# Alexandre-nk-Perdereau/video-fingerprint

Hardware: NVIDIA B200
Metric: fingerprint videos/s (64 frames@64^2) (higher is better)
Workload: dtype bf16

## Files before the change

### video_fingerprint_b200/csrc/vfp_b200.cu

```cuda
#include "../../include/vfp_b200.h"

#include <math.h>
#include <string.h>

#include <map>
#include <mutex>
#include <string>
#include <vector>

#include "conv1_kernel.cuh"
#include "attention_tc_kernel.cuh"
#include "conv3_ts_kernel.cuh"
#include "ffn_kernel.cuh"
#include "gemm_launch.cuh"
#include "join_kernels.cuh"
#include "metrics_kernels.cuh"
#include "model3d_kernels.cuh"
#include "preprocess_kernels.cuh"
#include "stem_ts_kernel.cuh"
#include "token_kernels.cuh"
#include "topk_kernels.cuh"

using namespace vfp;

namespace {

thread_local std::string g_last_error;

int fail(const std::string& msg) {
  g_last_error = msg;
  return 1;
}
int fail_cuda(const char* what, cudaError_t e) {
  g_last_error = std::string(what) + ": " + cudaGetErrorString(e);
  return 2;
}
#define VFP_CUDA(call)                                  \
  do {                                                  \
    cudaError_t e__ = (call);                           \
    if (e__ != cudaSuccess) return fail_cuda(#call, e__); \
  } while (0)

inline size_t align_up(size_t x, size_t a) { return (x + a - 1) / a * a; }

constexpr float kBnEps = 1e-5f;

enum Stage : int {
  kStConv1 = 0, kStConv2, kStConv3, kStConv4, kStTokEmbed, kStTemporalConv, kStLayerNorm, kStQkv, kStAttention,
  kStOutProj, kStMlp1, kStMlp2, kStPoolGemm, kStPool, kStFinal, kStMisc, kStStemFused, kStFfn, kNumStages
};
const char* const kStageNames[kNumStages] = {"conv1_stem", "conv2_igemm", "conv3_igemm", "conv4_igemm_pool", "token_embed_gemm",
                                             "temporal_conv", "layernorm", "qkv_gemm", "attention", "out_proj_gemm",
                                             "mlp1_gemm_gelu", "mlp2_gemm", "pool_logits_gemm", "temporal_pool",
                                             "final_projection", "misc", "stem_fused", "ffn_fused"};
struct Profiler {
  bool enabled = false;
  std::vector<cudaEvent_t> pool;
  std::vector<std::pair<int, cudaEvent_t>> marks;
  size_t next = 0;
  double ms[kNumStages] = {0};
  unsigned long long launches = 0;
  void mark(int stage, cudaStream_t st) {
    if (!enabled) return;
    if (next == pool.size()) {
      cudaEvent_t e;
      cudaEventCreate(&e);
      pool.push_back(e);
    }
    cudaEvent_t e = pool[next++];
    cudaEventRecord(e, st);
    marks.emplace_back(stage, e);
  }
  void drain() {
    if (marks.empty()) return;
    cudaEventSynchronize(marks.back().second);
    for (size_t i = 1; i < marks.size(); ++i) {
      if (marks[i].first < 0) continue;
      float t = 0.f;
      cudaEventElapsedTime(&t, marks[i - 1].second, marks[i].second);
      ms[marks[i].first] += t;
    }
    marks.clear();
    next = 0;
  }
};
Profiler g_prof;
const int kTemporalKernels[4] = {3, 5, 7, 11};

struct Conv2KBlock { int c_half, dw, dh; };
const Conv2KBlock kConv2KBlocks[6] = {{1, 0, -1}, {0, 0, 0}, {1, 0, 0}, {1, -1, -1}, {0, -1, 0}, {1, -1, 0}};
inline int conv2_tap_index(int d, int sub) { return d == -1 ? (sub == 1 ? 0 : -1) : (sub == 0 ? 1 : 2); }

struct AttnBlockWeights {
  float *ln1_w, *ln1_b, *ln2_w, *ln2_b;
  __nv_bfloat16 *wqkv, *wo, *w1, *w2;
  float *bqkv, *bo, *b1, *b2;
  CUtensorMap tm_qkv, tm_o, tm_w1, tm_w2;
  CUtensorMap tm_qkv_h, tm_o_h;
  CUtensorMap tm_w1_ffn, tm_w2_ffn;
};

}

struct vfp_weights {
  int embedding_dim = 0;
  int n_attn = 0;
  std::vector<void*> allocs;
  uint32_t* c1_wpack = nullptr;
  float* c1_bias = nullptr;
  __nv_bfloat16 *c2_w = nullptr, *c3_w = nullptr, *c4_w = nullptr;
  float *c2_b = nullptr, *c3_b = nullptr, *c4_b = nullptr;
  CUtensorMap tm_c2, tm_c3, tm_c4;
  CUtensorMap tm_c3h, tm_c4h;
  __nv_bfloat16* c2f_w = nullptr;
  CUtensorMap tm_c2f;
  __nv_bfloat16* c1ts_w = nullptr;
  CUtensorMap tm_c1ts;
  __nv_bfloat16* wtok = nullptr;
  float* btok = nullptr;
  float* pe = nullptr;
  int pe_len = 0;
  CUtensorMap tm_tok;
  float* tc_w[2] = {nullptr, nullptr};
  float* tc_b[2] = {nullptr, nullptr};
  std::vector<AttnBlockWeights> attn;
  __nv_bfloat16* wpool = nullptr;
  float* bpool = nullptr;
  CUtensorMap tm_pool;
  float *w0t = nullptr, *b0 = nullptr, *w3t = nullptr, *b3 = nullptr;
  bool head_on_tensor_cores = false;
  __nv_bfloat16 *w0_bf = nullptr, *w3_bf = nullptr;
  CUtensorMap tm_head0, tm_head3;
};

namespace {

struct TensorTable {
// ... 11 lines not shown
    }
    return static_cast<const float*>(it->second->data);
  }
  bool has(const std::string& name) const { return by_name.count(name) != 0; }
  int64_t numel(const std::string& name) const {
    auto it = by_name.find(name);
    return it == by_name.end() ? -1 : it->second->numel;
  }
};

template <class T>
int upload(vfp_weights* w, const std::vector<T>& host, T** dev) {
  void* p = nullptr;
  VFP_CUDA(cudaMalloc(&p, host.size() * sizeof(T)));
  w->allocs.push_back(p);
  VFP_CUDA(cudaMemcpy(p, host.data(), host.size() * sizeof(T), cudaMemcpyHostToDevice));
  *dev = static_cast<T*>(p);
  return 0;
}

std::vector<__nv_bfloat16> to_bf16(const std::vector<float>& v) {
  std::vector<__nv_bfloat16> o(v.size());
  for (size_t i = 0; i < v.size(); ++i) o[i] = __float2bfloat16(v[i]);
  return o;
}

struct BnFold {
  std::vector<float> scale, shift;
};
bool load_bn(const TensorTable& t, const std::string& prefix, int c, BnFold* out, std::string* err) {
  const float* g = t.get(prefix + ".weight", c, err);
  const float* b = g ? t.get(prefix + ".bias", c, err) : nullptr;
  const float* m = b ? t.get(prefix + ".running_mean", c, err) : nullptr;
  const float* v = m ? t.get(prefix + ".running_var", c, err) : nullptr;
  if (!v) return false;
  out->scale.resize(c);
  out->shift.resize(c);
  for (int i = 0; i < c; ++i) {
    const double s = (double)g[i] / sqrt((double)v[i] + (double)kBnEps);
    out->scale[i] = (float)s;
    out->shift[i] = (float)((double)b[i] - (double)m[i] * s);
  }
  return true;
}

int prep_conv3x3(vfp_weights* w, const TensorTable& t, int conv_idx, int cin, int cout, __nv_bfloat16** dw, float** db,
                 std::string* err) {
  const std::string p = "spatial_encoder.encoder.";
  const float* cw = t.get(p + std::to_string(conv_idx) + ".weight", (int64_t)cout * cin * 9, err);
  const float* cb = cw ? t.get(p + std::to_string(conv_idx) + ".bias", cout, err) : nullptr;
  BnFold bn;
  if (!cb || !load_bn(t, p + std::to_string(conv_idx + 1), cout, &bn, err)) return 1;
  std::vector<float> wf((size_t)cout * 9 * cin), bf(cout);
  for (int co = 0; co < cout; ++co) {
    for (int c = 0; c < cin; ++c)
      for (int kh = 0; kh < 3; ++kh)
        for (int kw = 0; kw < 3; ++kw)
          wf[(size_t)co * 9 * cin + (kh * 3 + kw) * cin + c] = cw[(((size_t)co * cin + c) * 3 + kh) * 3 + kw] * bn.scale[co];
    bf[co] = cb[co] * bn.scale[co] + bn.shift[co];
  }
  if (upload(w, to_bf16(wf), dw) || upload(w, bf, db)) return 1;
  return 0;
}

int prep_dense_bf16(vfp_weights* w, const float* src, size_t n, __nv_bfloat16** dev) {
  std::vector<float> v(src, src + n);
  return upload(w, to_bf16(v), dev);
}
int prep_f32(vfp_weights* w, const float* src, size_t n, float** dev) {
  std::vector<float> v(src, src + n);
  return upload(w, v, dev);
}

constexpr int64_t kConvPassFrames = 262144;
constexpr int64_t kStemPassFrames = 16384;
int64_t g_conv_pass_frames = 65536;
int64_t g_stem_pass_frames = kStemPassFrames;
int g_fused_stem = 2;
int g_join_prefetch = 16;
int g_attention_tc = 1;
int g_conv3_ts = 1;
int g_pair_gemm = 1;
int g_ffn_mode = 1;
int g_conv_mcast = 0;
int g_join_kernel = 2;
int g_join_symmetric = 1;
int g_join_panel_tiles = 512;

struct TokenWs {
  size_t cu, att_items, tok_pos, tok_len, feat, xa, xb, xn, qkv, att, delta, delta2, h, logits, xbf, pooled, pooled_bf, head_h, total;
};
struct ConvWs {
  size_t c1, c2, c3, total;
};
TokenWs token_ws_layout(int64_t F, int64_t C) {
  TokenWs L{};
  size_t off = 0;
  auto take = [&](size_t bytes) {
    const size_t o = off;
    off = align_up(off + bytes, 1024);
    return o;
  };
  L.cu = take((size_t)(C + 1) * 4);
  L.att_items = take((size_t)(F / 64 + C + 1) * 16);
  L.tok_pos = take((size_t)F * 4);
  L.tok_len = take((size_t)F * 4);
  L.feat = take((size_t)F * 256 * 2);
  L.xa = take((size_t)F * kDim * 4);
  L.xb = take((size_t)F * kDim * 4);
  L.xn = take((size_t)F * kDim * 2);
  L.qkv = take((size_t)F * 3 * kDim * 2);
  L.att = take((size_t)F * kDim * 2);
  L.delta = take((size_t)F * kDim * 2);
  L.delta2 = take((size_t)F * kDim * 2);
  L.h = take((size_t)F * 4 * kDim * 2);
  L.logits = take((size_t)F * kDim * 4);
  L.xbf = take((size_t)F * kDim * 2);
  L.pooled = take((size_t)C * 3 * kDim * 4);
  L.pooled_bf = take((size_t)C * 3 * kDim * 2);
  L.head_h = take((size_t)C * kDim * 2);
  L.total = off;
  return L;
}
ConvWs conv_ws_layout(int64_t F) {
  ConvWs L{};
  size_t off = 0;
  auto take = [&](size_t bytes) {
    const size_t o = off;
    off = align_up(off + bytes, 1024);
    return o;
  };
  L.c1 = take((size_t)std::min<int64_t>(F, kStemPassFrames) * 32 * 32 * 32 * 2);
  L.c2 = take((size_t)F * 16 * 16 * 64 * 2);
  L.c3 = take((size_t)F * 8 * 8 * 128 * 2);
  L.total = off;
  return L;
}
size_t forward_ws_total(int64_t F, int64_t C) {
  return token_ws_layout(F, C).total + conv_ws_layout(std::min<int64_t>(F, g_conv_pass_frames)).total;
}

constexpr int kMaxPipes = 4;
int g_forward_pipes = 1;

int pipe_streams(int n, cudaStream_t* out) {
  static std::mutex mu;
  static cudaStream_t pool[kMaxDevices][kMaxPipes] = {};
  std::lock_guard<std::mutex> g(mu);
  const int dev = current_device();
  for (int i = 0; i < n; ++i) {
    if (!pool[dev][i]) VFP_CUDA(cudaStreamCreateWithFlags(&pool[dev][i], cudaStreamNonBlocking));
    out[i] = pool[dev][i];
  }
  return 0;
}

}

extern "C" {

int vfp_abi_version(void) { return VFP_ABI_VERSION; }
const char* vfp_last_error(void) { return g_last_error.c_str(); }

int vfp_device_sm_count(void) {
  int n = 0, dev = 0;
  if (cudaGetDeviceCount(&n) != cudaSuccess || n <= 0) return 0;
  if (cudaGetDevice(&dev) != cudaSuccess) return 0;
  int sms = 0;
  if (cudaDeviceGetAttribute(&sms, cudaDevAttrMultiProcessorCount, dev) != cudaSuccess) return 0;
  return sms;
}

int vfp_set_tuning(int key, long long value) {
  if (key == 0 && value >= 64 && value <= kStemPassFrames) { g_stem_pass_frames = value; return 0; }
  if (key == 1 && (value == 0 || value == 2)) { g_fused_stem = (int)value; return 0; }
  if (key == 5 && value >= 0 && value <= 4096) { g_join_prefetch = (int)value; return 0; }
  if (key == 6 && value >= 0 && value <= 4096) { g_topk_prefetch = (int)value; return 0; }
  if (key == 3 && value >= 64 && value <= kConvPassFrames) { g_conv_pass_frames = value; return 0; }
  if (key == 16 && value >= 0 && value <= 1) { g_conv3_ts = (int)value; return 0; }
  if (key == 17 && value >= 0 && value <= 1) { g_attention_tc = (int)value; return 0; }
  if (key == 15 && value >= 0 && value <= 3) { g_pair_gemm = (int)value; return 0; }
  if (key == 14 && value >= 0 && value <= 1) { g_ffn_mode = (int)value; return 0; }
  if (key == 13 && value >= 0 && value <= 3) { g_conv_mcast = (int)value; return 0; }
  if (key == 10 && value >= 0 && value <= 2) { g_join_kernel = (int)value; return 0; }
  if (key == 11 && value >= 0 && value <= 1) { g_join_symmetric = (int)value; return 0; }
  if (key == 12 && value >= 16 && value <= 65536) { g_join_panel_tiles = (int)value; return 0; }
  if (key == 7 && value >= 0 && value <= 1) { pdl_enabled().store((int)value); return 0; }
  if (key == 8 && value >= 0 && value <= 4096) { persistent_cta_limit().store((int)value); return 0; }
  if (key == 9 && value >= 1 && value <= kMaxPipes) { g_forward_pipes = (int)value; return 0; }
  if (key == 2) {
    const int mode = value != 0;
    const unsigned int zero = 0;
    if (cudaMemcpyToSymbol(g_vfp_hang_mode, &mode, sizeof(mode)) != cudaSuccess) return 2;
    if (cudaMemcpyToSymbol(g_vfp_hang_count, &zero, sizeof(zero)) != cudaSuccess) return 2;
    return 0;
  }
  return 1;
}

int vfp_profile_enable(int on) {
  g_prof.drain();
  g_prof.enabled = on != 0;
  return 0;
}
int vfp_profile_num_stages(void) { return kNumStages; }
const char* vfp_profile_stage_name(int i) { return (i >= 0 && i < kNumStages) ? kStageNames[i] : ""; }
int vfp_profile_read(double* stage_ms, int n_stages, uint64_t* launches, int reset) {
  g_prof.drain();
  for (int i = 0; i < n_stages && i < kNumStages; ++i) stage_ms[i] = g_prof.ms[i];
  if (launches) *launches = g_prof.launches;
  if (reset) {
    for (int i = 0; i < kNumStages; ++i) g_prof.ms[i] = 0;
    g_prof.launches = 0;
  }
  return 0;
}

unsigned int vfp_device_error_word(void) {
  unsigned int v = 0, zero = 0;
  cudaDeviceSynchronize();
  cudaMemcpyFromSymbol(&v, g_vfp_device_error, sizeof(v));
  if (v) cudaMemcpyToSymbol(g_vfp_device_error, &zero, sizeof(zero));
  return v;
}

#ifdef VFP_FFN_TRACE
int vfp_debug_ffn_trace(long long* out, int max_pairs) {
  (void)max_pairs;
  cudaDeviceSynchronize();
  cudaMemcpyFromSymbol(out, g_ffn_trace, sizeof(long long) * 8192 / 2);
  static long long zeros[4096];
  cudaMemcpyToSymbol(g_ffn_trace, zeros, sizeof(zeros));
  return 2048;
}
#endif

int vfp_debug_hang_log(unsigned int* out, int max_entries) {
  unsigned int n = 0;
  cudaDeviceSynchronize();
  if (cudaMemcpyFromSymbol(&n, g_vfp_hang_count, sizeof(n)) != cudaSuccess) return -1;
  if (n > 64) n = 64;
  if ((int)n > max_entries) n = (unsigned int)max_entries;
  if (n && cudaMemcpyFromSymbol(out, g_vfp_hang_log, (size_t)n * 16) != cudaSuccess) return -1;
  return (int)n;
}

void vfp_weights_destroy(vfp_weights* w) {
  if (!w) return;
  for (void* p : w->allocs) cudaFree(p);
  delete w;
}

int vfp_weights_embedding_dim(const vfp_weights* w) { return w ? w->embedding_dim : 0; }

int vfp_weights_create(const vfp_tensor_desc* tensors, int n_tensors, vfp_weights** out) {
  if (!tensors || !out) return fail("vfp_weights_create: null argument");
  if (vfp_device_sm_count() <= 0) return fail("vfp_weights_create: no CUDA device (there is no CPU fallback)");
  if (!tensor_map_encoder()) return fail("vfp_weights_create: cuTensorMapEncodeTiled not available from the driver");
  TensorTable t;
  for (int i = 0; i < n_tensors; ++i) t.by_name[tensors[i].name] = &tensors[i];
  std::string err;
  vfp_weights* w = new vfp_weights();
  auto bail = [&](const std::string& m) {
    vfp_weights_destroy(w);
    return fail("vfp_weights_create: " + (m.empty() ? g_last_error : m));
// ... 247 lines not shown
      for (int kb = 0; kb < 6; ++kb) {
        s.tap_c_blk[kb] = (signed char)kConv2KBlocks[kb].c_half;
        s.tap_w[kb] = (signed char)kConv2KBlocks[kb].dw;
        s.tap_h[kb] = (signed char)kConv2KBlocks[kb].dh;
      }
      EpiBiasActTma<true>::Params ep{};
      if (make_tmap_out(&ep.tmap_out, c2a + (size_t)s0 * 256 * 64, (uint64_t)n * 256, 64, true)) return fail("tensor map encode failed (conv2 out)");
      ep.bias = w->c2_b; ep.N = 64; ep.act = 1;
      VFP_CUDA((launch_gemm<64, 64, 3, EpiBiasActTma<true>, 3>(ta, w->tm_c2, s, ep, st)));
      g_prof.mark(kStConv2, st);
    }
  }
  g_prof.launches += 2;
  {
    if (g_conv3_ts) {
      Conv3Params cp{};
      if (make_tmap_nhwc_bf16(&cp.tmap_in, c2a, F, 16, 16, 64, 64, 8, 8, kC3Frames, 2) || make_tmap_out(&cp.tmap_out, c3a, (uint64_t)F * 64, 128, true))
        return fail("tensor map encode failed (conv3)");
      cp.w = w->c3_w; cp.bias = w->c3_b; cp.n_tiles = (int)((F + kC3Frames - 1) / kC3Frames);
      VFP_CUDA(ensure_dynamic_smem(reinterpret_cast<const void*>(conv3_ts_kernel<7>), Conv3Smem<7>::kTotal));
      VFP_CUDA(launch_kernel(conv3_ts_kernel<7>, dim3(std::min(cp.n_tiles, persistent_grid())), dim3(kC3Threads), Conv3Smem<7>::kTotal, st, cp));
      g_prof.mark(kStConv3, st);
    } else {
    if (make_tmap_nhwc_bf16(&ta, c2a, F, 16, 16, 64, 64, 8, 8, 2, 2)) return fail("tensor map encode failed (conv3)");
    GemmShape s{};
    s.m_tiles = (int)((F + 1) / 2); s.n_tiles = 1; s.k_blocks = 9; s.group_m = 16; s.a_conv = 1;
    s.tiles_per_frame = 1; s.frames_per_tile = 2; s.tile_out_rows = 8;
    conv_taps_strided(&s, 1);
    EpiConvTransposedTma::Params ep{};
    if (make_tmap_out(&ep.tmap_out, c3a, (uint64_t)F * 64, 128, true)) return fail("tensor map encode failed (conv3 out)");
    ep.bias = w->c3_b; ep.c_out = 128; ep.pixels_per_tile = 256;
    if (g_conv_mcast & 1) VFP_CUDA((launch_gemm<128, 64, 4, EpiConvTransposedTma, 2, true, 2>(ta, w->tm_c3h, s, ep, st)));
    else VFP_CUDA((launch_gemm<128, 64, 4, EpiConvTransposedTma, 2, true>(ta, w->tm_c3, s, ep, st)));
    g_prof.mark(kStConv3, st);
    }
  }
  {
    if (make_tmap_nhwc_bf16(&ta, c3a, F, 8, 8, 128, 64, 4, 4, 8, 2)) return fail("tensor map encode failed (conv4)");
    GemmShape s{};
    s.m_tiles = (int)((F + 7) / 8); s.n_tiles = 1; s.k_blocks = 18; s.group_m = 16; s.a_conv = 1;
    s.tiles_per_frame = 1; s.frames_per_tile = 8; s.tile_out_rows = 4;
    conv_taps_strided(&s, 2);
    EpiConvPool16::Params ep{};
    ep.bias = w->c4_b; ep.out_bf16 = feat_out; ep.frames = (int)F; ep.N = 256;
    if (g_pair_gemm & 1) VFP_CUDA((launch_gemm_pair<64, 6, EpiConvPool16>(ta, w->tm_c4h, s, ep, st)));
    else if (g_conv_mcast & 2) VFP_CUDA((launch_gemm<256, 64, 4, EpiConvPool16, 1, false, 2>(ta, w->tm_c4h, s, ep, st)));
    else VFP_CUDA((launch_gemm<256, 64, 4, EpiConvPool16>(ta, w->tm_c4, s, ep, st)));
    g_prof.mark(kStConv4, st);
  }
  return 0;
}

int forward_pass(const vfp_weights* w, const uint8_t* frames_base, int frame_dtype, size_t frame_bytes,
                 const int32_t* cu_host, int c0, int c1, float* emb_out, float* features_out, uint8_t* ws,
                 cudaStream_t st) {
  const int C = c1 - c0;
  const int64_t f0 = cu_host[c0];
  const int64_t F = cu_host[c1] - f0;
  const TokenWs L = token_ws_layout(F, C);
  uint8_t* conv_ws = ws + L.total;
  int* d_cu = reinterpret_cast<int*>(ws + L.cu);
  int* tok_pos = reinterpret_cast<int*>(ws + L.tok_pos);
  int* tok_len = reinterpret_cast<int*>(ws + L.tok_len);
  __nv_bfloat16* feat = reinterpret_cast<__nv_bfloat16*>(ws + L.feat);
  float* xa = reinterpret_cast<float*>(ws + L.xa);
  float* xb = reinterpret_cast<float*>(ws + L.xb);
  __nv_bfloat16* xn = reinterpret_cast<__nv_bfloat16*>(ws + L.xn);
  __nv_bfloat16* qkv = reinterpret_cast<__nv_bfloat16*>(ws + L.qkv);
  __nv_bfloat16* att = reinterpret_cast<__nv_bfloat16*>(ws + L.att);
  __nv_bfloat16* delta = reinterpret_cast<__nv_bfloat16*>(ws + L.delta);
  __nv_bfloat16* delta_f = reinterpret_cast<__nv_bfloat16*>(ws + L.delta2);
  __nv_bfloat16* hbuf = reinterpret_cast<__nv_bfloat16*>(ws + L.h);
  float* logits = reinterpret_cast<float*>(ws + L.logits);
  __nv_bfloat16* xbf = reinterpret_cast<__nv_bfloat16*>(ws + L.xbf);
  float* pooled = reinterpret_cast<float*>(ws + L.pooled);
  __nv_bfloat16* pooled_bf = reinterpret_cast<__nv_bfloat16*>(ws + L.pooled_bf);
  __nv_bfloat16* head_h = reinterpret_cast<__nv_bfloat16*>(ws + L.head_h);

  std::vector<int32_t> cu_rel(C + 1);
  int max_T = 0;
  for (int i = 0; i <= C; ++i) cu_rel[i] = (int32_t)(cu_host[c0 + i] - f0);
  for (int i = 0; i < C; ++i) max_T = std::max(max_T, cu_rel[i + 1] - cu_rel[i]);
  g_prof.mark(-1, st);
  g_prof.launches += 8 + 7 * (unsigned long long)w->n_attn;
  VFP_CUDA(cudaMemcpyAsync(d_cu, cu_rel.data(), (size_t)(C + 1) * 4, cudaMemcpyHostToDevice, st));
  std::vector<int32_t> items_host;
  items_host.reserve((size_t)(F / kAttRows + C) * 4);
  for (int i = 0; i < C; ++i)
    for (int q = cu_rel[i]; q < cu_rel[i + 1]; q += kAttRows) {
      items_host.push_back(q); items_host.push_back(cu_rel[i]); items_host.push_back(cu_rel[i + 1]); items_host.push_back(0);
    }
  const size_t n_items = items_host.size() / 4;
  int4* att_items = reinterpret_cast<int4*>(ws + L.att_items);
  VFP_CUDA(cudaMemcpyAsync(att_items, items_host.data(), items_host.size() * 4, cudaMemcpyHostToDevice, st));
  VFP_CUDA(launch_kernel(token_map_kernel, dim3((unsigned)((F + 255) / 256)), dim3(256), 0, st, d_cu, C, (int)F, tok_pos, tok_len));
  g_prof.mark(kStMisc, st);

  for (int64_t s0 = 0; s0 < F; s0 += g_conv_pass_frames) {
    const int64_t n = std::min<int64_t>(g_conv_pass_frames, F - s0);
    if (int rc = encode_frames_pass(w, frames_base + (size_t)(f0 + s0) * frame_bytes, frame_dtype, n, feat + s0 * 256, conv_ws, st))
      return rc;
  }
  auto token_gemm = [&](const __nv_bfloat16* A, int64_t M, int K, const CUtensorMap& tb, int N, const EpiBiasAct::Params& ep) -> int {
    CUtensorMap tma;
    if (make_tmap_rows_bf16(&tma, A, (uint64_t)M, (uint64_t)K, (uint64_t)K, 128, 64)) return fail("tensor map encode failed (tokens)");
    GemmShape s = plain_shape(M, N, K, 256, 64, 32);
    if (K == 256) {
      VFP_CUDA((launch_gemm_bres<256, 64, 4, 4, EpiBiasAct>(tma, tb, s, ep, st)));
    } else {
      VFP_CUDA((launch_gemm<256, 64, 4, EpiBiasAct>(tma, tb, s, ep, st)));
    }
    return 0;
  };
  auto token_gemm_bf16 = [&](const __nv_bfloat16* A, int64_t M, int K, const CUtensorMap& tb, int N, const float* bias, int act,
                             __nv_bfloat16* out, const CUtensorMap* tb_half = nullptr) -> int {
    CUtensorMap tma;
    if (make_tmap_rows_bf16(&tma, A, (uint64_t)M, (uint64_t)K, (uint64_t)K, 128, 64)) return fail("tensor map encode failed (tokens)");
    EpiBiasActTma<true>::Params ep{};
    if (make_tmap_out(&ep.tmap_out, out, (uint64_t)M, (uint64_t)N, true)) return fail("tensor map encode failed (token out)");
    ep.bias = bias; ep.N = N; ep.act = act;
    GemmShape s = plain_shape(M, N, K, 256, 64, 32);
    if (tb_half && (g_pair_gemm & 2)) {
      VFP_CUDA((launch_gemm_pair<64, 6, EpiBiasActTma<true>>(tma, *tb_half, s, ep, st)));
    } else if (K == 256) {
      VFP_CUDA((launch_gemm_bres<256, 64, 4, 4, EpiBiasActTma<true>>(tma, tb, s, ep, st)));
    } else {
      VFP_CUDA((launch_gemm<256, 64, 4, EpiBiasActTma<true>>(tma, tb, s, ep, st)));
    }
    return 0;
  };
  {
    CUtensorMap tma;
    if (make_tmap_rows_bf16(&tma, feat, (uint64_t)F, 256, 256, 128, 64)) return fail("tensor map encode failed (tokens)");
    EpiBiasActTma<false>::Params ep{};
    if (make_tmap_out(&ep.tmap_out, xa, (uint64_t)F, kDim, false)) return fail("tensor map encode failed (token embedding out)");
    ep.bias = w->btok; ep.N = kDim; ep.act = 0; ep.pe = w->pe; ep.token_pos = tok_pos; ep.M = (int)F;
    GemmShape s = plain_shape(F, kDim, 256, 256, 64, 32);
    VFP_CUDA((launch_gemm_bres<256, 64, 2, 4, EpiBiasActTma<false>>(tma, w->tm_tok, s, ep, st)));
    g_prof.mark(kStTokEmbed, st);
  }
  {
    VFP_CUDA(ensure_dynamic_smem(reinterpret_cast<const void*>(temporal_conv_tma_kernel), kTc2SmemBytes));
    float* bufs[3] = {xa, xb, xa};
    for (int blk = 0; blk < 2; ++blk) {
      TemporalConvParams tp{};
      if (make_tmap_rows_f32(&tp.tmap_x, bufs[blk], (uint64_t)F, kDim, kTc2Rows)) return fail("tensor map encode failed (temporal conv)");
      tp.tok_pos = tok_pos; tp.tok_len = tok_len; tp.w = w->tc_w[blk]; tp.bias = w->tc_b[blk]; tp.y = bufs[blk + 1];
      tp.n_tokens = (int)F; tp.n_tiles = (int)((F + kTc2Tok - 1) / kTc2Tok);
      const int grid = std::min(tp.n_tiles, 2 * persistent_grid());
      VFP_CUDA(launch_kernel(temporal_conv_tma_kernel, dim3((unsigned)grid), dim3(kTc2Threads), kTc2SmemBytes, st, tp));
    }
    g_prof.mark(kStTemporalConv, st);
  }
  const unsigned ln_grid = (unsigned)((F * 32 + 255) / 256);
  VFP_CUDA(ensure_dynamic_smem(reinterpret_cast<const void*>(attention_fa_kernel), kAttSmemBytes));
  AttnTcParams atc{};
  if (g_attention_tc) {
    if (make_tmap_rows_bf16(&atc.tmap_qkv, qkv, (uint64_t)F, 3 * kDim, 3 * kDim, 64, 64)) return fail("tensor map encode failed (attention)");
    atc.items = att_items; atc.out = att; atc.n_units = (int)n_items * 4;
    VFP_CUDA(ensure_dynamic_smem(reinterpret_cast<const void*>(attention_tc_kernel), kAtcSmemBytes));
  }
  for (int b = 0; b < w->n_attn; ++b) {
    const AttnBlockWeights& a = w->attn[b];
    VFP_CUDA(launch_kernel(add_layernorm_bf16_kernel, dim3(ln_grid), dim3(256), 0, st, xa, b > 0 ? delta : nullptr, b > 0 ? delta_f : nullptr, a.ln1_w, a.ln1_b, xn, (int)F, 1));
    g_prof.mark(kStLayerNorm, st);
    if (token_gemm_bf16(xn, F, kDim, a.tm_qkv, 3 * kDim, a.bqkv, 0, qkv, &a.tm_qkv_h)) return 1;
    g_prof.mark(kStQkv, st);
    if (g_attention_tc) {
      const int grid = std::min(atc.n_units, 2 * persistent_grid());
      VFP_CUDA(launch_kernel(attention_tc_kernel, dim3((unsigned)grid), dim3(kAtcThreads), kAtcSmemBytes, st, atc));
    } else {
      VFP_CUDA(launch_kernel(attention_fa_kernel, dim3((unsigned)n_items), dim3(kAttThreads), kAttSmemBytes, st, qkv, att_items, att, (int)F));
    }
    g_prof.mark(kStAttention, st);
    if (token_gemm_bf16(att, F, kDim, a.tm_o, kDim, a.bo, 0, delta, &a.tm_o_h)) return 1;
    g_prof.mark(kStOutProj, st);
    VFP_CUDA(launch_kernel(add_layernorm_bf16_kernel, dim3(ln_grid), dim3(256), 0, st, xa, delta, (const __nv_bfloat16*)nullptr, a.ln2_w, a.ln2_b, xn, (int)F, 0));
    g_prof.mark(kStLayerNorm, st);
    if (g_ffn_mode == 0) {
      if (token_gemm_bf16(xn, F, kDim, a.tm_w1, 4 * kDim, a.b1, 2, hbuf)) return 1;
      g_prof.mark(kStMlp1, st);
      if (token_gemm_bf16(hbuf, F, 4 * kDim, a.tm_w2, kDim, a.b2, 0, delta_f)) return 1;
      g_prof.mark(kStMlp2, st);
    } else {
      FfnParams fp{};
      if (make_tmap_rows_bf16(&fp.tmap_x, xn, (uint64_t)F, kDim, kDim, 128, 64)) return fail("tensor map encode failed (feed-forward)");
      fp.tmap_w1 = a.tm_w1_ffn; fp.tmap_w2 = a.tm_w2_ffn;
      if (make_tmap_out(&fp.tmap_out, delta_f, (uint64_t)F, kDim, true)) return fail("tensor map encode failed (feed-forward out)");
      fp.b1 = a.b1; fp.b2 = a.b2; fp.M = (int)F; fp.pair_tiles = (int)((F + 255) / 256);
      const int grid = 2 * std::min(fp.pair_tiles, persistent_grid() / 2);
      VFP_CUDA(ensure_dynamic_smem(reinterpret_cast<const void*>(ffn_pair_kernel<5>), FfnSmem<5>::kTotal));
      VFP_CUDA(launch_kernel_cluster(2, ffn_pair_kernel<5>, dim3(grid), dim3(kFfnThreads), FfnSmem<5>::kTotal, st, fp));
      g_prof.mark(kStFfn, st);
    }
  }
  VFP_CUDA(launch_kernel(add_convert_bf16_kernel, dim3((unsigned)((F * kDim / 8 + 255) / 256)), dim3(256), 0, st, xa, w->n_attn > 0 ? delta : nullptr,
                         w->n_attn > 0 ? delta_f : nullptr, xbf, (long long)(F * kDim / 8)));
  if (features_out)
    VFP_CUDA(cudaMemcpyAsync(features_out + (size_t)f0 * kDim, xa, (size_t)F * kDim * 4, cudaMemcpyDeviceToDevice, st));
  {
    CUtensorMap tma;
    if (make_tmap_rows_bf16(&tma, xbf, (uint64_t)F, kDim, kDim, 128, 64)) return fail("tensor map encode failed (pool in)");
    EpiBiasActTma<false>::Params ep{};
    if (make_tmap_out(&ep.tmap_out, logits, (uint64_t)F, kDim, false)) return fail("tensor map encode failed (pool logits)");
    ep.bias = w->bpool; ep.N = kDim; ep.act = 1;
    GemmShape s = plain_shape(F, kDim, kDim, 256, 64, 32);
    VFP_CUDA((launch_gemm_bres<256, 64, 2, 4, EpiBiasActTma<false>>(tma, w->tm_pool, s, ep, st)));
    g_prof.mark(kStPoolGemm, st);
  }
  VFP_CUDA(launch_kernel(temporal_pool_kernel, dim3((unsigned)C), dim3(256), 0, st, xa, logits, d_cu, pooled, pooled_bf));
  g_prof.mark(kStPool, st);
  float* emb_dst = emb_out + (size_t)c0 * w->embedding_dim;
  if (w->head_on_tensor_cores) {
    EpiBiasAct::Params ep{};
    ep.bias = w->b0; ep.act = 1; ep.out_bf16 = head_h; ep.ld_out = kDim; ep.M = C; ep.N = kDim;
    if (token_gemm(pooled_bf, C, 3 * kDim, w->tm_head0, kDim, ep)) return 1;
    CUtensorMap tma;
    if (make_tmap_rows_bf16(&tma, head_h, (uint64_t)C, kDim, kDim, 128, 64)) return fail("tensor map encode failed (head)");
    GemmShape s = plain_shape(C, w->embedding_dim, kDim, 256, 64, 32);
    EpiBiasL2Norm::Params en{};
    en.bias = w->b3; en.out_f32 = emb_dst; en.M = C; en.N = w->embedding_dim;
    VFP_CUDA((launch_gemm<256, 64, 4, EpiBiasL2Norm>(tma, w->tm_head3, s, en, st)));
  } else {
    VFP_CUDA(launch_kernel(final_projection_kernel<8>, dim3((unsigned)((C + 7) / 8)), dim3(256), 0, st, pooled, w->w0t, w->b0, w->w3t, w->b3,
                           w->embedding_dim, C, emb_dst));
  }
  g_prof.mark(kStFinal, st);
  if (g_prof.marks.size() > 4096) g_prof.drain();
  VFP_CUDA(cudaGetLastError());
  return 0;
}

}

extern "C" {

int vfp_forward(const vfp_weights* w, const void* frames, int frame_dtype, const int32_t* cu, int n_clips,
                float* emb_out, float* features_out, void* workspace, size_t workspace_bytes, void* stream) {
  if (!w || !frames || !cu || !emb_out || !workspace) return fail("vfp_forward: null argument");
  if (n_clips <= 0) return fail("vfp_forward: n_clips must be positive");
  if (frame_dtype < 0 || frame_dtype > 3) return fail("vfp_forward: unknown frame dtype");
  const size_t frame_bytes = (size_t)12288 * (frame_dtype == VFP_FRAME_BF16 ? 2 : frame_dtype == VFP_FRAME_F32 ? 4 : 1);
  if (cu[0] != 0) return fail("vfp_forward: cu_seqlens[0] must be 0");
  int max_T = 0;
  for (int i = 0; i < n_clips; ++i) {
    const int T = cu[i + 1] - cu[i];
    if (T <= 0) return fail("vfp_forward: clip " + std::to_string(i) + " has no frames");
    if (T > w->pe_len)
      return fail("vfp_forward: clip " + std::to_string(i) + " has " + std::to_string(T) + " frames; the positional table holds " +
                  std::to_string(w->pe_len));
    max_T = std::max(max_T, T);
  }
  const int64_t total = cu[n_clips];
  auto fit = [&](size_t bytes) {
    int64_t lo = 0, hi = total;
    while (lo < hi) {
      const int64_t mid = (lo + hi + 1) / 2;
      if (forward_ws_total(mid, std::min<int64_t>(mid, n_clips)) <= bytes) lo = mid; else hi = mid - 1;
    }
    return lo;
  };
  int n_pipes = g_prof.enabled ? 1 : std::max(1, std::min(g_forward_pipes, kMaxPipes));
  n_pipes = (int)std::min<int64_t>(n_pipes, std::max<int64_t>(1, total / kConvPassFrames));
  auto slice_bytes = [&](int n) { return workspace_bytes / n / 1024 * 1024; };
  while (n_pipes > 1 && fit(slice_bytes(n_pipes)) < max_T) --n_pipes;
  const int64_t pass_frames = fit(slice_bytes(n_pipes));
  if (pass_frames < max_T)
    return fail("vfp_forward: workspace of " + std::to_string(workspace_bytes) + " bytes cannot hold the longest clip (" +
                std::to_string(max_T) + " frames need " + std::to_string(forward_ws_total(max_T, 1)) + ")");
  const size_t slice = slice_bytes(n_pipes);
  int64_t n_pass = (total + pass_frames - 1) / pass_frames;
  n_pass = (n_pass + n_pipes - 1) / n_pipes * n_pipes;
  const int64_t target = (total + n_pass - 1) / n_pass;
  cudaStream_t caller = static_cast<cudaStream_t>(stream);
  cudaStream_t pipe[kMaxPipes] = {caller, nullptr, nullptr, nullptr};
  cudaEvent_t fork = nullptr;
  if (n_pipes > 1) {
    if (int rc = pipe_streams(n_pipes, pipe)) return rc;
    VFP_CUDA(cudaEventCreateWithFlags(&fork, cudaEventDisableTiming));
    VFP_CUDA(cudaEventRecord(fork, caller));
// ... 553 lines not shown
```

Baseline: 300,000.

## Fuse attention out-projection, residual LayerNorm, FFN and next LN1 into one kernel

Adds a persistent 2-CTA cluster tcgen05 kernel. It runs the attention output projection, adds the residual into x, applies LayerNorm2, runs the fused FFN, then adds the second residual and applies the next block's LayerNorm1, or for the last block emits the bf16 features. This replaces the out-proj GEMM, the add+LN launch, the FFN kernel, the next LN1 launch and the final add_convert, cutting four launches per block and the round trips of the delta and xn tensors through global memory. In exchange the kernel is long and depends on delicate mbarrier phase tracking. It also reuses the A0 smem buffer for the LN2 output, which adds synchronisation points.

New measurement: 301,700, median of 6. No clear change (+0.6%).

```diff
diff --git a/video_fingerprint_b200/csrc/attn_tail_kernel.cuh b/video_fingerprint_b200/csrc/attn_tail_kernel.cuh
--- /dev/null
+++ b/video_fingerprint_b200/csrc/attn_tail_kernel.cuh
@@ -0,0 +1,432 @@
+#pragma once
+#include "ffn_kernel.cuh"
+#include "stem_common.cuh"
+#include "token_kernels.cuh"
+
+namespace vfp {
+
+template <int SLOTS>
+struct AttnTailSmem {
+  static constexpr int kA0 = 0;
+  static constexpr int kRing = kA0 + 4 * 16384;
+  static constexpr int kH = kRing + SLOTS * 16384;
+  static constexpr int kVec = kH + 4 * 16384;
+  static constexpr int kBars = kVec + 2048 * 4;
+  static constexpr int kTotal = kBars + 512 + 1024;
+};
+
+struct AttnTailParams {
+  alignas(64) CUtensorMap tmap_att;
+  alignas(64) CUtensorMap tmap_wo;
+  alignas(64) CUtensorMap tmap_w1;
+  alignas(64) CUtensorMap tmap_w2;
+  const float* bo;
+  const float* b1;
+  const float* b2;
+  const float* ln2_w;
+  const float* ln2_b;
+  const float* ln1n_w;
+  const float* ln1n_b;
+  float* x;
+  __nv_bfloat16* xn;
+  __nv_bfloat16* xbf;
+  int M;
+  int pair_tiles;
+};
+
+__device__ __forceinline__ uint4 layernorm_row_bf16(float (&v)[8], const float* gamma, const float* beta, int lane) {
+  float s = 0.f;
+#pragma unroll
+  for (int i = 0; i < 8; ++i) s += v[i];
+#pragma unroll
+  for (int o = 16; o > 0; o >>= 1) s += __shfl_xor_sync(0xffffffffu, s, o);
+  const float mean = s * (1.0f / kDim);
+  float q = 0.f;
+#pragma unroll
+  for (int i = 0; i < 8; ++i) { v[i] -= mean; q += v[i] * v[i]; }
+#pragma unroll
+  for (int o = 16; o > 0; o >>= 1) q += __shfl_xor_sync(0xffffffffu, q, o);
+  const float rstd = rsqrtf(q * (1.0f / kDim) + 1e-5f);
+  const float4 g0 = reinterpret_cast<const float4*>(gamma)[lane * 2];
+  const float4 g1 = reinterpret_cast<const float4*>(gamma)[lane * 2 + 1];
+  const float4 b0 = reinterpret_cast<const float4*>(beta)[lane * 2];
+  const float4 b1 = reinterpret_cast<const float4*>(beta)[lane * 2 + 1];
+  uint4 o;
+  o.x = pack_bf16x2(v[0] * rstd * g0.x + b0.x, v[1] * rstd * g0.y + b0.y);
+  o.y = pack_bf16x2(v[2] * rstd * g0.z + b0.z, v[3] * rstd * g0.w + b0.w);
+  o.z = pack_bf16x2(v[4] * rstd * g1.x + b1.x, v[5] * rstd * g1.y + b1.y);
+  o.w = pack_bf16x2(v[6] * rstd * g1.z + b1.z, v[7] * rstd * g1.w + b1.w);
+  return o;
+}
+
+template <int SLOTS>
+__global__ void __launch_bounds__(kFfnThreads, 1) attn_tail_pair_kernel(const __grid_constant__ AttnTailParams p) {
+  using L = AttnTailSmem<SLOTS>;
+  static_assert(L::kTotal <= 232448, "attention tail kernel shared memory");
+  extern __shared__ uint8_t smem_raw[];
+  uint8_t* smem = smem_raw + ((1024u - (smem_u32(smem_raw) & 1023u)) & 1023u);
+  uint8_t* a0 = smem + L::kA0;
+  uint8_t* ring = smem + L::kRing;
+  uint8_t* hbuf = smem + L::kH;
+  float* svec = reinterpret_cast<float*>(smem + L::kVec);
+  uint32_t* sb1_h = reinterpret_cast<uint32_t*>(svec);
+  float* sb2 = svec + 512;
+  float* sbo = svec + 768;
+  float* sg2 = svec + 1024;
+  float* sbe2 = svec + 1280;
+  float* sg1n = svec + 1536;
+  float* sbe1n = svec + 1792;
+  uint64_t* bars = reinterpret_cast<uint64_t*>(smem + L::kBars);
+  uint64_t* full = bars;
+  uint64_t* empty = bars + SLOTS;
+  uint64_t* a0_full = bars + 2 * SLOTS;
+  uint64_t* a0_empty = a0_full + 1;
+  uint64_t* d1_full = a0_full + 2;
+  uint64_t* d1_empty = a0_full + 3;
+  uint64_t* h_full = a0_full + 4;
+  uint64_t* h_empty = a0_full + 5;
+  uint64_t* d2_full = a0_full + 6;
+  uint64_t* d2_empty = a0_full + 7;
+  uint32_t* tmem_slot = reinterpret_cast<uint32_t*>(a0_full + 8);
+
+  const int warp = threadIdx.x >> 5, lane = threadIdx.x & 31;
+  const uint32_t crank = cluster_ctarank();
+  const bool leader = crank == 0;
+  const int pair = blockIdx.x >> 1, n_pairs = gridDim.x >> 1;
+  const int my_tiles = p.pair_tiles > pair ? (p.pair_tiles - pair + n_pairs - 1) / n_pairs : 0;
+  const int n_chunks = my_tiles * kFfnChunks;
+  pdl_launch_dependents();
+
+  if (warp == 0 && lane == 0) {
+    tma_prefetch_desc(&p.tmap_att);
+    tma_prefetch_desc(&p.tmap_wo);
+    tma_prefetch_desc(&p.tmap_w1);
+    tma_prefetch_desc(&p.tmap_w2);
+    for (int i = 0; i < SLOTS; ++i) {
+      mbar_init(&full[i], 1);
+      mbar_init(&empty[i], 1);
+    }
+    mbar_init(a0_full, 1);
+    mbar_init(a0_empty, 1);
+    mbar_init(d1_full, 1);
+    mbar_init(d1_empty, 2 * kFfnActWarps);
+    mbar_init(h_full, 2 * kFfnActWarps);
+    mbar_init(h_empty, 1);
+    mbar_init(d2_full, 1);
+    mbar_init(d2_empty, 2 * kFfnActWarps);
+    fence_mbar_init();
+  }
+  if (warp == 1) {
+    tmem_alloc_2cta(tmem_slot, 512);
+    tmem_relinquish_2cta();
+  }
+  for (int i = threadIdx.x; i < kFfnHidden / 2; i += kFfnThreads) {
+    const __half2 h = __floats2half2_rn(__ldg(p.b1 + 2 * i), __ldg(p.b1 + 2 * i + 1));
+    sb1_h[i] = *reinterpret_cast<const uint32_t*>(&h);
+  }
+  for (int i = threadIdx.x; i < kDim; i += kFfnThreads) {
+    sb2[i] = __ldg(p.b2 + i);
+    sbo[i] = __ldg(p.bo + i);
+    sg2[i] = __ldg(p.ln2_w + i);
+    sbe2[i] = __ldg(p.ln2_b + i);
+    sg1n[i] = p.ln1n_w ? __ldg(p.ln1n_w + i) : 0.f;
+    sbe1n[i] = p.ln1n_b ? __ldg(p.ln1n_b + i) : 0.f;
+  }
+  tc_fence_before();
+  __syncthreads();
+  cluster_sync_all();
+  tc_fence_after();
+  const uint32_t tmem_base = *tmem_slot;
+  pdl_wait();
+
+  if (warp == 0) {
+    if (lane == 0) {
+      int slot = 0;
+      uint32_t ph = 0, a_ph = 0;
+      const uint32_t a0_full_leader = mapa_u32(a0_full, 0);
+      auto load_w = [&](const CUtensorMap* map, int k_col, int row0) {
+        mbar_wait(&empty[slot], ph ^ 1);
+        if (leader) mbar_arrive_expect_tx(&full[slot], 2 * 16384);
+        tma_load_2d_2cta(map, mapa_u32(&full[slot], 0), ring + slot * 16384, k_col, row0 + (int)crank * 128);
+        if (++slot == SLOTS) { slot = 0; ph ^= 1; }
+      };
+      auto prefetch_tile = [&](int tile) {
+        if (tile >= p.pair_tiles) return;
+        const int row0 = (tile * 2 + (int)crank) * 128;
+        for (int kb = 0; kb < 4; ++kb) tma_prefetch_l2_2d(&p.tmap_att, kb * 64, row0);
+        for (int r = row0; r < row0 + 128 && r < p.M; r += 16)
+          bulk_prefetch_l2(p.x + (size_t)r * kDim, (uint32_t)(min(16, p.M - r) * kDim * 4));
+      };
+      auto load_op = [&](int tile) {
+        prefetch_tile(tile + n_pairs);
+        mbar_wait(a0_empty, a_ph ^ 1);
+        a_ph ^= 1;
+        if (leader) mbar_arrive_expect_tx(a0_full, 2 * 4 * 16384);
+        for (int kb = 0; kb < 4; ++kb) tma_load_2d_2cta(&p.tmap_att, a0_full_leader, a0 + kb * 16384, kb * 64, (tile * 2 + (int)crank) * 128);
+        for (int kb = 0; kb < 4; ++kb) load_w(&p.tmap_wo, kb * 64, 0);
+      };
+      auto load_g1 = [&](int n) {
+        for (int kb = 0; kb < 4; ++kb) load_w(&p.tmap_w1, kb * 64, (n % kFfnChunks) * kFfnChunk);
+      };
+      auto load_g2 = [&](int n) {
+        for (int kb = 0; kb < 4; ++kb) load_w(&p.tmap_w2, (n % kFfnChunks) * kFfnChunk + kb * 64, 0);
+      };
+      if (n_chunks > 0) { prefetch_tile(pair); load_op(pair); load_g1(0); }
+      for (int n = 0; n < n_chunks; ++n) {
+        const bool more = n + 1 < n_chunks;
+        if (n % kFfnChunks == kFfnChunks - 1) {
+          if (more) load_op(pair + ((n + 1) / kFfnChunks) * n_pairs);
+          load_g2(n);
+          if (more) load_g1(n + 1);
+        } else {
+          load_g1(n + 1);
+          load_g2(n);
+        }
+      }
+    }
+  } else if (warp == 1) {
+    if (lane == 0 && leader) {
+      constexpr uint32_t idesc = umma_idesc_bf16(256, 256);
+      int slot = 0;
+      uint32_t ph = 0, a_ph = 0, d1e_ph = 0, hf_ph = 0, d2e_ph = 0;
+      const uint32_t a0_addr = smem_u32(a0), h_addr = smem_u32(hbuf);
+      auto commit_slot = [&]() {
+        umma_commit_2cta(&empty[slot], 3);
+        if (++slot == SLOTS) { slot = 0; ph ^= 1; }
+      };
+      auto d1_gemm = [&](uint32_t a_base) {
+        mbar_wait(d1_empty, d1e_ph ^ 1);
+        d1e_ph ^= 1;
+        tc_fence_after();
+        for (int kb = 0; kb < 4; ++kb) {
+          mbar_wait(&full[slot], ph);
+          tc_fence_after();
+          const uint64_t adesc = umma_smem_desc_kmajor<128>(a_base + kb * 16384);
+          const uint64_t bdesc = umma_smem_desc_kmajor<128>(smem_u32(ring + slot * 16384));
+#pragma unroll
+          for (int k = 0; k < 4; ++k) umma_bf16_2cta(tmem_base, adesc + 2 * k, bdesc + 2 * k, idesc, (kb | k) != 0 ? 1u : 0u);
+          commit_slot();
+        }
+        umma_commit_2cta(d1_full, 3);
+      };
+      auto out_proj = [&]() {
+        mbar_wait(a0_full, a_ph);
+        a_ph ^= 1;
+        d1_gemm(a0_addr);
+      };
+      auto gemm1 = [&](int n) {
+        d1_gemm(a0_addr);
+        if (n % kFfnChunks == kFfnChunks - 1) umma_commit_2cta(a0_empty, 3);
+      };
+      auto gemm2 = [&](int n) {
+        const int c = n % kFfnChunks;
+        if (c == 0) {
+          mbar_wait(d2_empty, d2e_ph ^ 1);
+          d2e_ph ^= 1;
+        }
+        mbar_wait(h_full, hf_ph);
+        hf_ph ^= 1;
+        tc_fence_after();
+        for (int kb = 0; kb < 4; ++kb) {
+          mbar_wait(&full[slot], ph);
+          tc_fence_after();
+          const uint64_t adesc = umma_smem_desc_kmajor<128>(h_addr + kb * 16384);
+          const uint64_t bdesc = umma_smem_desc_kmajor<128>(smem_u32(ring + slot * 16384));
+#pragma unroll
+          for (int k = 0; k < 4; ++k) umma_bf16_2cta(tmem_base + 256, adesc + 2 * k, bdesc + 2 * k, idesc, (c | kb | k) != 0 ? 1u : 0u);
+          commit_slot();
+        }
+        umma_commit_2cta(h_empty, 3);
+        if (c == kFfnChunks - 1) umma_commit_2cta(d2_full, 3);
+      };
+      if (n_chunks > 0) { out_proj(); gemm1(0); }
+      for (int n = 0; n < n_chunks; ++n) {
+        const bool more = n + 1 < n_chunks;
+        if (n % kFfnChunks == kFfnChunks - 1) {
+          if (more) out_proj();
+          gemm2(n);
+          if (more) gemm1(n + 1);
+        } else {
+          gemm1(n + 1);
+          gemm2(n);
+        }
+      }
+    }
+  } else {
+    const int q = warp & 3;
+    const int cq = (warp - 2) >> 2;
+    const int row = q * 32 + lane;
+    const int rbase = (warp - 2) * 8;
+    const uint32_t lane_addr = tmem_base + (static_cast<uint32_t>(q * 32) << 16);
+    uint32_t d1f_ph = 0, he_ph = 0, d2f_ph = 0;
+    const uint32_t d1_empty_leader = mapa_u32(d1_empty, 0), h_full_leader = mapa_u32(h_full, 0), d2_empty_leader = mapa_u32(d2_empty, 0);
+    const uint32_t sw = (uint32_t)(row & 7);
+    const int koff = cq * 16384 + row * 128;
+    auto row_piece = [&](int r) { return (lane >> 3) * 16384 + r * 128 + (((lane & 7) ^ (r & 7)) << 4); };
+
+    auto stage_delta = [&](uint32_t taddr, const float* bias, uint8_t* dst) {
+#pragma unroll
+      for (int cc = 0; cc < 2; ++cc) {
+        uint32_t v[32];
+        tmem_ld_32x32(taddr + cq * 64 + cc * 32, v);
+        tmem_ld_wait();
+#pragma unroll
+        for (int pc = 0; pc < 4; ++pc) {
+          const float* b = bias + cq * 64 + cc * 32 + 8 * pc;
+          const float4 ba = *reinterpret_cast<const float4*>(b);
+          const float4 bc = *reinterpret_cast<const float4*>(b + 4);
+          uint4 o;
+          o.x = pack_bf16x2(__uint_as_float(v[8 * pc + 0]) + ba.x, __uint_as_float(v[8 * pc + 1]) + ba.y);
+          o.y = pack_bf16x2(__uint_as_float(v[8 * pc + 2]) + ba.z, __uint_as_float(v[8 * pc + 3]) + ba.w);
+          o.z = pack_bf16x2(__uint_as_float(v[8 * pc + 4]) + bc.x, __uint_as_float(v[8 * pc + 5]) + bc.y);
+          o.w = pack_bf16x2(__uint_as_float(v[8 * pc + 6]) + bc.z, __uint_as_float(v[8 * pc + 7]) + bc.w);
+          *reinterpret_cast<uint4*>(dst + koff + (((cc * 4 + pc) ^ sw) << 4)) = o;
+        }
+      }
+    };
+    auto load_x = [&](long long grow0, int j, float4 (&xr)[2]) {
+      const long long g = grow0 + rbase + j;
+      if (g < p.M) {
+        const float4* src = reinterpret_cast<const float4*>(p.x + g * kDim) + lane * 2;
+        xr[0] = src[0];
+        xr[1] = src[1];
+      } else {
+        xr[0] = xr[1] = make_float4(0.f, 0.f, 0.f, 0.f);
+      }
+    };
+    auto add_delta = [&](const float4 (&xr)[2], uint4 d, float (&v)[8]) {
+      v[0] = xr[0].x; v[1] = xr[0].y; v[2] = xr[0].z; v[3] = xr[0].w;
+      v[4] = xr[1].x; v[5] = xr[1].y; v[6] = xr[1].z; v[7] = xr[1].w;
+      const __nv_bfloat162* dp = reinterpret_cast<const __nv_bfloat162*>(&d);
+#pragma unroll
+      for (int e = 0; e < 4; ++e) {
+        const float2 f = __bfloat1622float2(dp[e]);
+        v[2 * e] += f.x;
+        v[2 * e + 1] += f.y;
+      }
+    };
+    auto store_x = [&](long long g, const float (&v)[8]) {
+      float4* dst = reinterpret_cast<float4*>(p.x + g * kDim) + lane * 2;
+      dst[0] = make_float4(v[0], v[1], v[2], v[3]);
+      dst[1] = make_float4(v[4], v[5], v[6], v[7]);
+    };
+    constexpr int kXDepth = 3;
+    auto epi_bar = [&]() { asm volatile("bar.sync 1, %0;" ::"n"(32 * kFfnActWarps) : "memory"); };
+
+    auto ln2_epilogue = [&](int tile) {
+      const long long grow0 = (long long)(tile * 2 + (int)crank) * 128;
+      float4 xr[kXDepth][2];
+#pragma unroll
+      for (int j = 0; j < kXDepth; ++j) load_x(grow0, j, xr[j]);
+      mbar_wait(d1_full, d1f_ph);
+      d1f_ph ^= 1;
+      tc_fence_after();
+      stage_delta(lane_addr, sbo, a0);
+      tc_fence_before();
+      epi_bar();
+#pragma unroll
+      for (int j = 0; j < 8; ++j) {
+        const int r = rbase + j;
+        uint4* piece = reinterpret_cast<uint4*>(a0 + row_piece(r));
+        float v[8];
+        add_delta(xr[j % kXDepth], *piece, v);
+        if (j + kXDepth < 8) load_x(grow0, j + kXDepth, xr[j % kXDepth]);
+        if (grow0 + r < p.M) store_x(grow0 + r, v);
+        *piece = layernorm_row_bf16(v, sg2, sbe2, lane);
+      }
+      fence_proxy_async_smem();
+      __syncwarp();
+      if (lane == 0) mbar_arrive_cluster(d1_empty_leader);
+    };
+    auto output_tile = [&](int tile) {
+      const long long grow0 = (long long)(tile * 2 + (int)crank) * 128;
+      float4 xr[kXDepth][2];
+#pragma unroll
+      for (int j = 0; j < kXDepth; ++j) load_x(grow0, j, xr[j]);
+      mbar_wait(d2_full, d2f_ph);
+      d2f_ph ^= 1;
+      tc_fence_after();
+      stage_delta(lane_addr + 256, sb2, hbuf);
+      tc_fence_before();
+      __syncwarp();
+      if (lane == 0) mbar_arrive_cluster(d2_empty_leader);
+      epi_bar();
+#pragma unroll
+      for (int j = 0; j < 8; ++j) {
+        const int r = rbase + j;
+        const long long g = grow0 + r;
+        float v[8];
+        add_delta(xr[j % kXDepth], *reinterpret_cast<const uint4*>(hbuf + row_piece(r)), v);
+        if (j + kXDepth < 8) load_x(grow0, j + kXDepth, xr[j % kXDepth]);
+        if (g < p.M) {
+          store_x(g, v);
+          uint4 o;
+          if (p.xn) {
+            o = layernorm_row_bf16(v, sg1n, sbe1n, lane);
+          } else {
+            o.x = pack_bf16x2(v[0], v[1]); o.y = pack_bf16x2(v[2], v[3]);
+            o.z = pack_bf16x2(v[4], v[5]); o.w = pack_bf16x2(v[6], v[7]);
+          }
+          reinterpret_cast<uint4*>((p.xn ? p.xn : p.xbf) + g * kDim)[lane] = o;
+        }
+      }
+      epi_bar();
+    };
+
+    for (int n = 0; n < n_chunks; ++n) {
+      const int c = n % kFfnChunks;
+      if (c == 0) {
+        const int j = n / kFfnChunks;
+        ln2_epilogue(pair + j * n_pairs);
+        if (j > 0) output_tile(pair + (j - 1) * n_pairs);
+      }
+      mbar_wait(d1_full, d1f_ph);
+      d1f_ph ^= 1;
+      tc_fence_after();
+      uint32_t packed[32];
+      {
+        uint32_t va[32], vb[32];
+        tmem_ld_32x32(lane_addr + cq * 64, va);
+        tmem_ld_32x32(lane_addr + cq * 64 + 32, vb);
+        tmem_ld_wait();
+        tc_fence_before();
+        __syncwarp();
+        if (lane == 0) mbar_arrive_cluster(d1_empty_leader);
+#pragma unroll
+        for (int cc = 0; cc < 2; ++cc) {
+          uint32_t(&v)[32] = cc ? vb : va;
+          const uint32_t* bias = sb1_h + (c * kFfnChunk + cq * 64 + cc * 32) / 2;
+#pragma unroll
+          for (int i = 0; i < 32; i += 8) {
+            const uint4 bb = *reinterpret_cast<const uint4*>(bias + i / 2);
+            packed[cc * 16 + i / 2] = gelu_bias_bf16x2(make_float2(__uint_as_float(v[i]), __uint_as_float(v[i + 1])), bb.x);
+            packed[cc * 16 + i / 2 + 1] = gelu_bias_bf16x2(make_float2(__uint_as_float(v[i + 2]), __uint_as_float(v[i + 3])), bb.y);
+            packed[cc * 16 + i / 2 + 2] = gelu_bias_bf16x2(make_float2(__uint_as_float(v[i + 4]), __uint_as_float(v[i + 5])), bb.z);
+            packed[cc * 16 + i / 2 + 3] = gelu_bias_bf16x2(make_float2(__uint_as_float(v[i + 6]), __uint_as_float(v[i + 7])), bb.w);
+          }
+        }
+      }
+      mbar_wait(h_empty, he_ph ^ 1);
+      he_ph ^= 1;
+#pragma unroll
+      for (int piece = 0; piece < 8; ++piece)
+        *reinterpret_cast<uint4*>(hbuf + koff + ((piece ^ sw) << 4)) =
+            make_uint4(packed[4 * piece], packed[4 * piece + 1], packed[4 * piece + 2], packed[4 * piece + 3]);
+      fence_proxy_async_smem();
+      __syncwarp();
+      if (lane == 0) mbar_arrive_cluster(h_full_leader);
+    }
+    if (n_chunks > 0) output_tile(pair + (my_tiles - 1) * n_pairs);
+  }
+
+  __syncwarp();
+  tc_fence_before();
+  __syncthreads();
+  cluster_sync_all();
+  if (warp == 1) {
+    tc_fence_after();
+    tmem_dealloc_2cta(tmem_base, 512);
+  }
+}
+
+}
diff --git a/video_fingerprint_b200/csrc/vfp_b200.cu b/video_fingerprint_b200/csrc/vfp_b200.cu
--- a/video_fingerprint_b200/csrc/vfp_b200.cu
+++ b/video_fingerprint_b200/csrc/vfp_b200.cu
@@ -10,6 +10,7 @@
 
 #include "conv1_kernel.cuh"
 #include "attention_tc_kernel.cuh"
+#include "attn_tail_kernel.cuh"
 #include "conv3_ts_kernel.cuh"
 #include "ffn_kernel.cuh"
 #include "gemm_launch.cuh"
@@ -47,12 +48,13 @@
 
 enum Stage : int {
   kStConv1 = 0, kStConv2, kStConv3, kStConv4, kStTokEmbed, kStTemporalConv, kStLayerNorm, kStQkv, kStAttention,
-  kStOutProj, kStMlp1, kStMlp2, kStPoolGemm, kStPool, kStFinal, kStMisc, kStStemFused, kStFfn, kNumStages
+  kStOutProj, kStMlp1, kStMlp2, kStPoolGemm, kStPool, kStFinal, kStMisc, kStStemFused, kStFfn, kStAttnTail, kNumStages
 };
 const char* const kStageNames[kNumStages] = {"conv1_stem", "conv2_igemm", "conv3_igemm", "conv4_igemm_pool", "token_embed_gemm",
                                              "temporal_conv", "layernorm", "qkv_gemm", "attention", "out_proj_gemm",
                                              "mlp1_gemm_gelu", "mlp2_gemm", "pool_logits_gemm", "temporal_pool",
-                                             "final_projection", "misc", "stem_fused", "ffn_fused"};
+                                             "final_projection", "misc", "stem_fused", "ffn_fused",
+                                             "attn_tail_fused"};
 struct Profiler {
   bool enabled = false;
   std::vector<cudaEvent_t> pool;
@@ -230,6 +232,7 @@
 int g_conv3_ts = 1;
 int g_pair_gemm = 1;
 int g_ffn_mode = 1;
+int g_attn_tail = 1;
 int g_conv_mcast = 0;
 int g_join_kernel = 2;
 int g_join_symmetric = 1;
@@ -329,6 +332,7 @@
   if (key == 17 && value >= 0 && value <= 1) { g_attention_tc = (int)value; return 0; }
   if (key == 15 && value >= 0 && value <= 3) { g_pair_gemm = (int)value; return 0; }
   if (key == 14 && value >= 0 && value <= 1) { g_ffn_mode = (int)value; return 0; }
+  if (key == 18 && value >= 0 && value <= 1) { g_attn_tail = (int)value; return 0; }
   if (key == 13 && value >= 0 && value <= 3) { g_conv_mcast = (int)value; return 0; }
   if (key == 10 && value >= 0 && value <= 2) { g_join_kernel = (int)value; return 0; }
   if (key == 11 && value >= 0 && value <= 1) { g_join_symmetric = (int)value; return 0; }
@@ -742,7 +746,8 @@
   for (int i = 0; i <= C; ++i) cu_rel[i] = (int32_t)(cu_host[c0 + i] - f0);
   for (int i = 0; i < C; ++i) max_T = std::max(max_T, cu_rel[i + 1] - cu_rel[i]);
   g_prof.mark(-1, st);
-  g_prof.launches += 8 + 7 * (unsigned long long)w->n_attn;
+  const bool fused_tail = g_attn_tail && g_ffn_mode == 1 && w->n_attn > 0;
+  g_prof.launches += fused_tail ? 8 + 3 * (unsigned long long)w->n_attn : 8 + 7 * (unsigned long long)w->n_attn;
   VFP_CUDA(cudaMemcpyAsync(d_cu, cu_rel.data(), (size_t)(C + 1) * 4, cudaMemcpyHostToDevice, st));
   std::vector<int32_t> items_host;
   items_host.reserve((size_t)(F / kAttRows + C) * 4);
@@ -820,10 +825,13 @@
     atc.items = att_items; atc.out = att; atc.n_units = (int)n_items * 4;
     VFP_CUDA(ensure_dynamic_smem(reinterpret_cast<const void*>(attention_tc_kernel), kAtcSmemBytes));
   }
+  if (fused_tail) VFP_CUDA(ensure_dynamic_smem(reinterpret_cast<const void*>(attn_tail_pair_kernel<5>), AttnTailSmem<5>::kTotal));
   for (int b = 0; b < w->n_attn; ++b) {
     const AttnBlockWeights& a = w->attn[b];
-    VFP_CUDA(launch_kernel(add_layernorm_bf16_kernel, dim3(ln_grid), dim3(256), 0, st, xa, b > 0 ? delta : nullptr, b > 0 ? delta_f : nullptr, a.ln1_w, a.ln1_b, xn, (int)F, 1));
-    g_prof.mark(kStLayerNorm, st);
+    if (b == 0 || !fused_tail) {
+      VFP_CUDA(launch_kernel(add_layernorm_bf16_kernel, dim3(ln_grid), dim3(256), 0, st, xa, b > 0 ? delta : nullptr, b > 0 ? delta_f : nullptr, a.ln1_w, a.ln1_b, xn, (int)F, 1));
+      g_prof.mark(kStLayerNorm, st);
+    }
     if (token_gemm_bf16(xn, F, kDim, a.tm_qkv, 3 * kDim, a.bqkv, 0, qkv, &a.tm_qkv_h)) return 1;
     g_prof.mark(kStQkv, st);
     if (g_attention_tc) {
@@ -833,6 +841,21 @@
       VFP_CUDA(launch_kernel(attention_fa_kernel, dim3((unsigned)n_items), dim3(kAttThreads), kAttSmemBytes, st, qkv, att_items, att, (int)F));
     }
     g_prof.mark(kStAttention, st);
+    if (fused_tail) {
+      const bool last = b + 1 == w->n_attn;
+      AttnTailParams tp{};
+      if (make_tmap_rows_bf16(&tp.tmap_att, att, (uint64_t)F, kDim, kDim, 128, 64)) return fail("tensor map encode failed (attention tail)");
+      tp.tmap_wo = a.tm_o_h; tp.tmap_w1 = a.tm_w1_ffn; tp.tmap_w2 = a.tm_w2_ffn;
+      tp.bo = a.bo; tp.b1 = a.b1; tp.b2 = a.b2; tp.ln2_w = a.ln2_w; tp.ln2_b = a.ln2_b;
+      tp.ln1n_w = last ? nullptr : w->attn[b + 1].ln1_w;
+      tp.ln1n_b = last ? nullptr : w->attn[b + 1].ln1_b;
+      tp.x = xa; tp.xn = last ? nullptr : xn; tp.xbf = last ? xbf : nullptr;
+      tp.M = (int)F; tp.pair_tiles = (int)((F + 255) / 256);
+      const int grid = 2 * std::min(tp.pair_tiles, persistent_grid() / 2);
+      VFP_CUDA(launch_kernel_cluster(2, attn_tail_pair_kernel<5>, dim3(grid), dim3(kFfnThreads), AttnTailSmem<5>::kTotal, st, tp));
+      g_prof.mark(kStAttnTail, st);
+      continue;
+    }
     if (token_gemm_bf16(att, F, kDim, a.tm_o, kDim, a.bo, 0, delta, &a.tm_o_h)) return 1;
     g_prof.mark(kStOutProj, st);
     VFP_CUDA(launch_kernel(add_layernorm_bf16_kernel, dim3(ln_grid), dim3(256), 0, st, xa, delta, (const __nv_bfloat16*)nullptr, a.ln2_w, a.ln2_b, xn, (int)F, 0));
@@ -854,8 +877,9 @@
       g_prof.mark(kStFfn, st);
     }
   }
-  VFP_CUDA(launch_kernel(add_convert_bf16_kernel, dim3((unsigned)((F * kDim / 8 + 255) / 256)), dim3(256), 0, st, xa, w->n_attn > 0 ? delta : nullptr,
-                         w->n_attn > 0 ? delta_f : nullptr, xbf, (long long)(F * kDim / 8)));
+  if (!fused_tail)
+    VFP_CUDA(launch_kernel(add_convert_bf16_kernel, dim3((unsigned)((F * kDim / 8 + 255) / 256)), dim3(256), 0, st, xa, w->n_attn > 0 ? delta : nullptr,
+                           w->n_attn > 0 ? delta_f : nullptr, xbf, (long long)(F * kDim / 8)));
   if (features_out)
     VFP_CUDA(cudaMemcpyAsync(features_out + (size_t)f0 * kDim, xa, (size_t)F * kDim * 4, cudaMemcpyDeviceToDevice, st));
   {
```
